# daihangpku/SW-NeRF

Measured on AMD Instinct MI355X. Metric: rays/sec (64+128 samples/ray), higher is better.
Workload: dtype f32

## Files before the change

### __graft_entry__.py

```python
import os
import subprocess
import sys

ROOT = os.path.dirname(os.path.abspath(__file__))
PKG = os.path.join(ROOT, "sw-nerf_amd")
CSRC = os.path.join(PKG, "csrc")
LIB = os.path.join(PKG, "swnerf", "libswnerf_hip.so")
SOURCES = ["render_kernels.hip", "train_kernels.hip", "misc_kernels.hip", "pack_kernels.hip", "backward_kernels.hip", "wgrad_kernels.hip", "wgrad_x3_kernels.hip", "generic_kernels.hip", "x3_kernels.hip", "mesh_kernels.hip", "tnerf_kernels.hip", "tnerf_train_kernels.hip", "metrics_kernels.hip", "pyramid_kernels.hip", "fit2d_kernels.hip", "batch_kernels.hip", "optim_kernels.hip", "patch_kernels.hip", "query_kernels.hip", "image_kernels.hip", "lpips_kernels.hip", "jpeg_kernels.hip", "jpeg_enc_kernels.hip", "marker_kernels.hip", "meshops_kernels.hip", "meshsimp_kernels.hip", "meshfill_kernels.hip"]
HEADERS = ["swnerf_common.h", "mlp_core.h", "mlp_core_x3.h", "bf16x3_split.h", "mlp_kernels.h", "render_pass.h", "composite.h", "resample.h", "wave_dpp.h", "lds_dma.h", "host_util.h", "wgrad_host.h", "mc_tables.h", "elu.h", "ray_rows.h", "tnerf_pass.h", "pyramid_interp.h", "jpeg_math.h", "jpeg_host.h", "jpeg_enc_math.h", "jpeg_enc_host.h", "marker_math.h", "meshops_math.h", "meshops_layout.h", "meshops_common.h", "par_prims.h", "fit2d_cols.h", os.path.join(ROOT, "include", "swnerf.h")]
HIPCC_FLAGS = ["--offload-arch=gfx950", "-O3", "-ffp-contract=off", "-fPIC", "-shared", "-std=c++17"]


OBJDIR = os.path.join(PKG, "build")


def _deps():
    return [os.path.join(CSRC, s) for s in SOURCES] + [h if os.path.isabs(h) else os.path.join(CSRC, h) for h in HEADERS]


def _stale():
    if not os.path.exists(LIB):
        return True
    t = os.path.getmtime(LIB)
    return any(os.path.getmtime(d) > t for d in _deps())


def compile_library(force=False):
    if not (force or _stale()):
        return False
    from concurrent.futures import ThreadPoolExecutor
    hipcc = os.environ.get("HIPCC", "/opt/rocm/bin/hipcc")
    os.makedirs(OBJDIR, exist_ok=True)
    newest_header = max(os.path.getmtime(h if os.path.isabs(h) else os.path.join(CSRC, h)) for h in HEADERS)
    jobs = []
    for s in SOURCES:
        src, obj = os.path.join(CSRC, s), os.path.join(OBJDIR, s.replace(".hip", ".o"))
        if force or not os.path.exists(obj) or os.path.getmtime(obj) < max(os.path.getmtime(src), newest_header):
            jobs.append([hipcc] + [f for f in HIPCC_FLAGS if f != "-shared"] + ["-c", src, "-o", obj])
    for cmd in jobs:
        print("[build]", " ".join(cmd), file=sys.stderr, flush=True)
    with ThreadPoolExecutor(max_workers=min(len(jobs), 6) or 1) as ex:
        for r in ex.map(lambda c: subprocess.run(c, cwd=CSRC), jobs):
            if r.returncode != 0:
                raise RuntimeError(f"hipcc failed: {' '.join(r.args)}")
    tmp = LIB + f".tmp{os.getpid()}"
    link = [hipcc, "--offload-arch=gfx950", "-fPIC", "-shared", "-o", tmp] + [os.path.join(OBJDIR, s.replace(".hip", ".o")) for s in SOURCES]
    print("[build]", " ".join(link), file=sys.stderr, flush=True)
    try:
        subprocess.run(link, check=True, cwd=CSRC)
        os.replace(tmp, LIB)
    finally:
        if os.path.exists(tmp):
            os.remove(tmp)
    return True


def compile_library_locked(force=False):
    if not (force or _stale()):
        return False
    import fcntl
    os.makedirs(OBJDIR, exist_ok=True)
    with open(os.path.join(OBJDIR, ".lock"), "w") as lk:
        fcntl.flock(lk, fcntl.LOCK_EX)
        try:
            return compile_library(force)
        finally:
            fcntl.flock(lk, fcntl.LOCK_UN)


def check_library():
    if _stale():
        raise RuntimeError(f"{LIB} is missing or older than its sources: run __graft_entry__.compile_library() before touching the GPU")
    if PKG not in sys.path:
        sys.path.insert(0, PKG)
    import swnerf
    from swnerf import _lib
    L = _lib.lib()
    missing = [n for n in _lib.EXPORTS if not hasattr(L, n)]
    if missing:
        raise RuntimeError(f"libswnerf_hip.so lacks symbols: {missing}")
    return L


def build(force=False):
    compile_library_locked(force)
    L = check_library()
    if ROOT not in sys.path:
        sys.path.insert(0, ROOT)
    import oracle.nerf_oracle
    print(f"[build] ok: {LIB} (version {L.swnerf_version()})", file=sys.stderr, flush=True)


# ... 49 lines not shown
```

### sw-nerf_amd/csrc/mlp_core.h

```cpp
#pragma once
#include <hip/hip_runtime.h>
#include "swnerf_common.h"
#include "lds_dma.h"

typedef float f32x16 __attribute__((ext_vector_type(16)));
typedef float f32x4 __attribute__((ext_vector_type(4)));

struct WStream {
    const char* base;
    unsigned voff;
    unsigned lds_addr;
    const float* ring;
    f32x4 a_cur;
    const float* bias;
    const char* cont;
};

template <int N>
__device__ __forceinline__ void ws_wait() {
    asm volatile("s_waitcnt vmcnt(%0)" :: "n"(N) : "memory");
}

__device__ __forceinline__ f32x4 ws_read(const WStream& ws, int slot) {
    return *reinterpret_cast<const f32x4*>(ws.ring + slot * SW_STEP_FLOATS);
}

template <int I>
__device__ __forceinline__ void ws_prime(WStream& ws) {
    if constexpr (I < SW_RING) {
        ws_dma(ws.base + I * 1024, ws.voff, ws.lds_addr + I * 1024);
        ws_prime<I + 1>(ws);
    }
}

__device__ __forceinline__ void ws_start(WStream& ws, const float* w, const float* lds_bias, float* lds_ring, int lane) {
    ws.base = reinterpret_cast<const char*>(w);
    ws.voff = (unsigned)lane * 16u;
    ws.lds_addr = __builtin_amdgcn_readfirstlane((unsigned)(size_t)lds_ring);
    ws.ring = lds_ring + lane * 4;
    ws.bias = lds_bias + (lane >> 5) * 16;
    ws_prime<0>(ws);
    ws_wait<SW_RING - 1>();
    ws.a_cur = ws_read(ws, 0);
}

__device__ __forceinline__ void ws_rewind(WStream& ws, const float* w, const float* lds_bias, int lane) {
    ws.base = reinterpret_cast<const char*>(w);
    ws.bias = lds_bias + (lane >> 5) * 16;
}

__device__ __forceinline__ void ws_restart(WStream& ws, const float* w) {
    asm volatile("s_waitcnt vmcnt(0)" ::: "memory");
    ws.base = reinterpret_cast<const char*>(w);
    ws_prime<0>(ws);
    ws_wait<SW_RING - 1>();
    ws.a_cur = ws_read(ws, 0);
}

enum { SEG_ACC = 0, SEG_BIAS = 1, SEG_ZERO = 2, SEG_BIAS_SCALED = 3 };
template <int INIT>
__device__ __forceinline__ void seg_init_read(f32x16& b, const WStream& ws, int n) {
    if constexpr (INIT == SEG_BIAS || INIT == SEG_BIAS_SCALED) {
#pragma unroll
        for (int g = 0; g < 4; ++g) {
            const f32x4 v = *reinterpret_cast<const f32x4*>(ws.bias + n * SW_BIAS_TILE_FLOATS + 4 * g);
            b[4 * g + 0] = v[0]; b[4 * g + 1] = v[1]; b[4 * g + 2] = v[2]; b[4 * g + 3] = v[3];
        }
    }
}

struct SideStore {
    float* sp;
    float* mp; f32x4 mv;
};

struct SideFetch {
    const char* base; unsigned voff, lds_addr;
};

template <int S, int NS, int NT, int KT, int INIT, int SK, int FK = 0, bool REDIR = false>
__device__ __forceinline__ void seg_steps(f32x16 (&out)[NT], const f32x16 (&kin)[KT], WStream& ws, f32x16& binit, float scale,
                                          const SideStore& ss, const SideFetch& sf = SideFetch{nullptr, 0u, 0u}) {
    if constexpr (S < NS) {
        constexpr int n = S / (KT * 4), kt = (S / 4) % KT, q = S % 4;
        constexpr int slot = S % SW_RING, nslot = (S + 1) % SW_RING;
        constexpr bool tile_first = (S % (KT * 4)) == 0, tile_last = ((S + 1) % (KT * 4)) == 0;
        if constexpr (tile_first) {
            if constexpr (INIT == SEG_BIAS) out[n] = binit;
            else if constexpr (INIT == SEG_BIAS_SCALED) out[n] = binit * scale;
            else if constexpr (INIT == SEG_ZERO) {
#pragma unroll
                for (int r = 0; r < 16; ++r) out[n][r] = 0.f;
            }
        }
        ws_wait<SW_RING - 2>();
        const f32x4 a_next = ws_read(ws, nslot);
        if constexpr (tile_last && n + 1 < NT) seg_init_read<INIT>(binit, ws, n + 1);
        __builtin_amdgcn_sched_barrier(0);
        const f32x4 a = ws.a_cur;
        out[n] = __builtin_amdgcn_mfma_f32_32x32x2f32(a[0], kin[kt][4 * q + 0], out[n], 0, 0, 0);
        out[n] = __builtin_amdgcn_mfma_f32_32x32x2f32(a[1], kin[kt][4 * q + 1], out[n], 0, 0, 0);
        out[n] = __builtin_amdgcn_mfma_f32_32x32x2f32(a[2], kin[kt][4 * q + 2], out[n], 0, 0, 0);
        out[n] = __builtin_amdgcn_mfma_f32_32x32x2f32(a[3], kin[kt][4 * q + 3], out[n], 0, 0, 0);
        __builtin_amdgcn_sched_barrier(0);
        if constexpr (REDIR && S + SW_RING >= NS) ws_dma(ws.cont + (S + SW_RING - NS) * 1024, ws.voff, ws.lds_addr + slot * 1024);
        else ws_dma(ws.base + (S + SW_RING) * 1024, ws.voff, ws.lds_addr + slot * 1024);
        if constexpr (SK > 0) {
            constexpr int total = 4 * SK, every = NS / total;
            static_assert(every >= 1, "segment too short for its side stores");
            if constexpr (S % every == every - 1 && S / every < total) {
                constexpr int idx = S / every, n2 = idx / 4, g = idx % 4;
                const f32x4 v = {kin[n2][4 * g], kin[n2][4 * g + 1], kin[n2][4 * g + 2], kin[n2][4 * g + 3]};
                *reinterpret_cast<f32x4*>(ss.sp + 32 * n2 + 8 * g) = v;
            }
            if constexpr (S == 1) {
                if (ss.mp) *reinterpret_cast<f32x4*>(ss.mp) = ss.mv;
            }
            __builtin_amdgcn_sched_barrier(0);
        }
        if constexpr (FK > 0) {
            constexpr int ftotal = 4 * FK, fevery = (NS - SW_RING) / ftotal;
            static_assert(fevery >= 1, "segment too short for its side fetches");
            if constexpr (S % fevery == 0 && S / fevery < ftotal) {
                constexpr int c = S / fevery;
                ws_dma(sf.base + (32 * (c >> 2) + 8 * (c & 3)) * 4, sf.voff, sf.lds_addr + c * 1024);
            }
        }
        ws.a_cur = a_next;
        seg_steps<S + 1, NS, NT, KT, INIT, SK, FK, REDIR>(out, kin, ws, binit, scale, ss, sf);
    }
}

template <int NT, int KT, int INIT, int SK = 0, int FK = 0, bool REDIR = false>
__device__ __forceinline__ void seg_mfma(f32x16 (&out)[NT], const f32x16 (&kin)[KT], WStream& ws, float scale = 1.f,
                                         const SideStore& ss = SideStore{nullptr, nullptr, {0.f, 0.f, 0.f, 0.f}},
                                         const SideFetch& sf = SideFetch{nullptr, 0u, 0u}) {
    constexpr int NS = NT * KT * 4;
    static_assert(NS % SW_RING == 0, "segment must keep the ring phase");
    f32x16 binit;
    seg_init_read<INIT>(binit, ws, 0);
    seg_steps<0, NS, NT, KT, INIT, SK, FK, REDIR>(out, kin, ws, binit, scale, ss, sf);
    if (INIT == SEG_BIAS || INIT == SEG_BIAS_SCALED) ws.bias += NT * SW_BIAS_TILE_FLOATS;
    if constexpr (REDIR) ws.base = ws.cont;
    else ws.base += NS * 1024;
}

#define SW_MASK_LAYERS 9
#define SW_MASK_TILE_FLOATS (SW_MASK_LAYERS * 256)
template <int NT>
__device__ __forceinline__ f32x4 relu_bits(const f32x16 (&t)[NT]) {
    unsigned m[4] = {0u, 0u, 0u, 0u};
#pragma unroll
    for (int n = 0; n < NT; ++n)
#pragma unroll
        for (int r = 0; r < 16; ++r) {
            const int b = min(max(__float_as_int(t[n][r]), 0), 1);
            m[n >> 1] |= (unsigned)b << (16 * (n & 1) + r);
        }
    f32x4 v = {__uint_as_float(m[0]), __uint_as_float(m[1]), __uint_as_float(m[2]), __uint_as_float(m[3])};
    return v;
}

template <int NT>
__device__ __forceinline__ void mask_apply(const f32x4& mv, f32x16 (&t)[NT]) {
#pragma unroll
    for (int n = 0; n < NT; ++n)
#pragma unroll
        for (int r = 0; r < 16; ++r) {
            const int m = __float_as_int(mv[n >> 1]);
            const int keep = (m << (31 - (16 * (n & 1) + r))) >> 31;
            t[n][r] = __int_as_float(__float_as_int(t[n][r]) & keep);
        }
}

__device__ __forceinline__ float relu1(float x) {
    float y;
    asm("v_max_f32_e32 %0, 0, %1" : "=v"(y) : "v"(x));
    return y;
}

template <int NOUT, int NT>
__device__ __forceinline__ void head_valu(const f32x16 (&x)[NT], WStream& ws, float (&res)[NOUT]) {
#pragma unroll
    for (int o = 0; o < NOUT; ++o) {
        float acc = 0.f;
#pragma unroll
        for (int n = 0; n < NT; ++n)
#pragma unroll
            for (int g = 0; g < 4; ++g) {
                const f32x4 w = *reinterpret_cast<const f32x4*>(ws.bias + (o * NT + n) * SW_BIAS_TILE_FLOATS + 4 * g);
                acc = fmaf(w[0], x[n][4 * g + 0], acc); acc = fmaf(w[1], x[n][4 * g + 1], acc);
                acc = fmaf(w[2], x[n][4 * g + 2], acc); acc = fmaf(w[3], x[n][4 * g + 3], acc);
            }
        res[o] = acc + __shfl_xor(acc, 32, 64);
        asm volatile("" : "+v"(res[o]));
    }
    ws.bias += NOUT * NT * SW_BIAS_TILE_FLOATS;
}

template <int NT>
__device__ __forceinline__ void head_valu_rt(const f32x16 (&x)[NT], WStream& ws, int nout, float (&res)[5]) {
#pragma nounroll
    for (int o = 0; o < nout; ++o) {
        float acc = 0.f;
#pragma unroll
        for (int n = 0; n < NT; ++n)
#pragma unroll
            for (int g = 0; g < 4; ++g) {
                const f32x4 w = *reinterpret_cast<const f32x4*>(ws.bias + (o * NT + n) * SW_BIAS_TILE_FLOATS + 4 * g);
                acc = fmaf(w[0], x[n][4 * g + 0], acc); acc = fmaf(w[1], x[n][4 * g + 1], acc);
                acc = fmaf(w[2], x[n][4 * g + 2], acc); acc = fmaf(w[3], x[n][4 * g + 3], acc);
            }
        float v = acc + __shfl_xor(acc, 32, 64);
        asm volatile("" : "+v"(v));
        res[0] = o == 0 ? v : res[0]; res[1] = o == 1 ? v : res[1]; res[2] = o == 2 ? v : res[2];
        res[3] = o == 3 ? v : res[3]; res[4] = o == 4 ? v : res[4];
    }
    ws.bias += nout * NT * SW_BIAS_TILE_FLOATS;
}

template <int NT>
__device__ __forceinline__ void tiles_store(float* rowp, const f32x16 (&t)[NT]) {
#pragma unroll
    for (int n = 0; n < NT; ++n)
#pragma unroll
        for (int g = 0; g < 4; ++g) {
            f32x4 v = {t[n][4 * g], t[n][4 * g + 1], t[n][4 * g + 2], t[n][4 * g + 3]};
            *reinterpret_cast<f32x4*>(rowp + 32 * n + 8 * g) = v;
        }
}

__device__ __forceinline__ void bias_to_lds(float* lds_bias, const float* gbias, int nfloats) {
    for (int i = threadIdx.x * 4; i < nfloats; i += blockDim.x * 4)
        *reinterpret_cast<f32x4*>(lds_bias + i) = *reinterpret_cast<const f32x4*>(gbias + i);
    __syncthreads();
}

__device__ __forceinline__ void pe_pos(float x0, float x1, float x2, int h, f32x16 (&e)[2]) {
#pragma unroll
    for (int a = 0; a < 32; ++a) {
        float v;
        if (a < 30) {
            const int k = a / 3, c = a % 3;
            const float xc = (c == 0) ? x0 : ((c == 1) ? x1 : x2);
            v = sw_sin_or_cos(xc * (float)(1 << k), h);
        } else if (a == 30) {
            v = h ? x2 : x0;
        } else {
            v = h ? 0.f : x1;
        }
        e[a >> 4][a & 15] = v;
    }
}

__device__ __forceinline__ void pe_dir(float d0, float d1, float d2, int h, f32x16& e) {
#pragma unroll
    for (int a = 0; a < 16; ++a) {
        float v = 0.f;
        if (a < 12) {
            const int k = a / 3, c = a % 3;
            const float dc = (c == 0) ? d0 : ((c == 1) ? d1 : d2);
            v = sw_sin_or_cos(dc * (float)(1 << k), h);
        } else if (a == 12) {
            v = h ? d2 : d0;
        } else if (a == 13) {
            v = h ? 0.f : d1;
        }
        e[a] = v;
    }
}

__device__ __forceinline__ void pe_time(float t, int h, f32x16& e) {
#pragma unroll
    for (int a = 0; a < 16; ++a) {
        float v = 0.f;
        if (a < 10) v = sw_sin_or_cos(t * (float)(1 << a), h);
        else if (a == 10) v = h ? 0.f : t;
        e[a] = v;
    }
}

#define SW_EMB_LDS_FLOATS (3 * 16 * 64)
__device__ __forceinline__ void emb_park(float* lds_emb, int lane, const f32x16 (&e)[2]) {
#pragma unroll
    for (int a = 0; a < 32; ++a) lds_emb[a * 64 + lane] = e[a >> 4][a & 15];
}
__device__ __forceinline__ void emb_fetch(const float* lds_emb, int lane, f32x16 (&e)[2]) {
#pragma unroll
    for (int a = 0; a < 32; ++a) e[a >> 4][a & 15] = lds_emb[a * 64 + lane];
}

__device__ __forceinline__ void tile_park(float* lds_tile, int lane, const f32x16& e) {
#pragma unroll
    for (int a = 0; a < 16; ++a) lds_tile[a * 64 + lane] = e[a];
}
__device__ __forceinline__ void tile_fetch(const float* lds_tile, int lane, f32x16& e) {
#pragma unroll
    for (int a = 0; a < 16; ++a) e[a] = lds_tile[a * 64 + lane];
}

template <bool DNERF, bool TRAIN = false, bool XS = false, bool NOHEAD = false, bool TB = false, bool REDIR = false>
__device__ __forceinline__ void trunk_pass(const f32x16 (&emb)[2], float* lds_emb, float t, bool deform_pass, int h,
                                           f32x16 (&in)[8], f32x16 (&out)[8], float (&head)[3], WStream& ws,
                                           float* act_row = nullptr, float* mask_tile = nullptr, bool store_last = false,
                                           f32x4* mb = nullptr, float* xs_row = nullptr, const float* lds_tb = nullptr,
                                           const char* cont7 = nullptr) {
    static_assert(!REDIR || (!TRAIN && !DNERF && !NOHEAD), "the redirect serves the static inference pass");
    const int lane_ = threadIdx.x & 63;
    emb_park(lds_emb, lane_, emb);
    f32x4 mbits = {0.f, 0.f, 0.f, 0.f};
#pragma nounroll
    for (int l = 0; l < 8; ++l) {
        if (l == 0) {
            if (DNERF && deform_pass) {
                if constexpr (TB) {
                    const float* keep = ws.bias;
                    ws.bias = lds_tb + (lane_ & 32 ? 16 : 0);
                    if (XS) {
                        seg_mfma<8, 2, SEG_BIAS, 2>(out, emb, ws, 1.f, SideStore{xs_row, nullptr, mbits});
                        f32x16 tt;
                        pe_time(t, h, tt);
#pragma unroll
                        for (int g = 0; g < 4; ++g) {
                            const f32x4 v = {tt[4 * g], tt[4 * g + 1], tt[4 * g + 2], tt[4 * g + 3]};
                            *reinterpret_cast<f32x4*>(xs_row + 64 + 8 * g) = v;
                        }
                    } else {
                        seg_mfma<8, 2, SEG_BIAS>(out, emb, ws);
                    }
                    ws.bias = keep;
                } else {
                    f32x16 k1[1];
                    pe_time(t, h, k1[0]);
                    seg_mfma<8, 1, SEG_BIAS>(out, k1, ws);
                    seg_mfma<8, 2, SEG_ACC>(out, emb, ws);
                }
            } else if (XS) {
                seg_mfma<8, 2, SEG_BIAS, 2>(out, emb, ws, 1.f, SideStore{xs_row, nullptr, mbits});
            } else {
                seg_mfma<8, 2, SEG_BIAS>(out, emb, ws);
            }
        } else {
            if (TRAIN) {
                const SideStore ss{act_row + 256 * (l - 1), mask_tile + 256 * (l - 1), mbits};
                seg_mfma<8, 8, SEG_BIAS, TRAIN ? 8 : 0>(out, in, ws, 1.f, ss);
            } else if constexpr (REDIR) {
                const char* next = ws.base + SW_STEPS_TRUNK * 1024;
                ws.cont = (l == 7 && cont7) ? cont7 : next;
                seg_mfma<8, 8, SEG_BIAS, 0, 0, true>(out, in, ws);
            } else {
                seg_mfma<8, 8, SEG_BIAS>(out, in, ws);
            }
            if (l == 5) {
                f32x16 e2[2];
                emb_fetch(lds_emb, lane_, e2);
                seg_mfma<8, 2, SEG_ACC>(out, e2, ws);
            }
        }
#pragma unroll
        for (int n = 0; n < 8; ++n)
#pragma unroll
            for (int r = 0; r < 16; ++r) in[n][r] = relu1(out[n][r]);
        if (TRAIN) mbits = relu_bits<8>(in);
    }
    if (TRAIN) {
        if (store_last) {
            tiles_store<8>(act_row + 256 * 7, in);
            *reinterpret_cast<f32x4*>(mask_tile + 256 * 7) = mbits;
        } else {
            *mb = mbits;
        }
    }
    if constexpr (NOHEAD) return;
    if (DNERF && deform_pass) {
        head_valu<3, 8>(in, ws, head);
        head[0] += ws.bias[0]; head[1] += ws.bias[1]; head[2] += ws.bias[2];
    } else {
        float s1[1];
        head_valu<1, 8>(in, ws, s1);
        head[0] = s1[0] + ws.bias[0]; head[1] = 0.f; head[2] = 0.f;
    }
    ws.bias += SW_BIAS_TILE_FLOATS;
}

#define SW_VB_LDS_FLOATS (4 * SW_BIAS_TILE_FLOATS)

__device__ __forceinline__ void view_bias_tile(const f32x16& demb, float* lds_vb, int lane, WStream& ws) {
    f32x16 k1[1], c[4];
    k1[0] = demb;
    seg_mfma<4, 1, SEG_BIAS>(c, k1, ws);
    if ((lane & 31) == 0) {
        float* o = lds_vb + (lane >> 5) * 16;
#pragma unroll
        for (int n = 0; n < 4; ++n)
#pragma unroll
            for (int g = 0; g < 4; ++g) {
                const f32x4 v = {c[n][4 * g], c[n][4 * g + 1], c[n][4 * g + 2], c[n][4 * g + 3]};
                *reinterpret_cast<f32x4*>(o + n * SW_BIAS_TILE_FLOATS + 4 * g) = v;
            }
    }
    __builtin_amdgcn_fence(__ATOMIC_ACQ_REL, "wavefront");
    __builtin_amdgcn_wave_barrier();
}

#define SW_TB_LDS_FLOATS (8 * SW_BIAS_TILE_FLOATS)
__device__ __forceinline__ void time_bias_tile(float t, int h, float* lds_tb, int lane, WStream& ws) {
    f32x16 k1[1], c[8];
    pe_time(t, h, k1[0]);
    seg_mfma<8, 1, SEG_BIAS>(c, k1, ws);
    if ((lane & 31) == 0) {
        float* o = lds_tb + (lane >> 5) * 16;
#pragma unroll
        for (int n = 0; n < 8; ++n)
#pragma unroll
            for (int g = 0; g < 4; ++g) {
                const f32x4 v = {c[n][4 * g], c[n][4 * g + 1], c[n][4 * g + 2], c[n][4 * g + 3]};
                *reinterpret_cast<f32x4*>(o + n * SW_BIAS_TILE_FLOATS + 4 * g) = v;
            }
    }
    __builtin_amdgcn_fence(__ATOMIC_ACQ_REL, "wavefront");
    __builtin_amdgcn_wave_barrier();
// ... 49 lines not shown
```

### sw-nerf_amd/csrc/render_pass.h

```cpp
#pragma once
#include <cstdlib>
#include "mlp_kernels.h"
#include "mlp_core_x3.h"
#include "resample.h"
#include "composite.h"
#include "ray_rows.h"

#define SW_LDS_SC 256
#define SW_LDS_SORT 1024
#define SW_LDS_WAVE_FLOATS (3 * SW_LDS_SC + SW_LDS_SORT)

#define SW_DEFER_SMAX 240
#define SW_DEFER_LDS_FLOATS (4 * SW_DEFER_SMAX + 64)
#define SW_DEFER_WS_FLOATS (64 * 256)
static_assert(SW_DEFER_LDS_FLOATS <= SW_LDS_SORT, "the deferred colour scratch shares the sort region");

struct PassDev {
    swnerf_pass_args a;
    const float* w0;
    const float* b0;
    int nbias;
    int two_pass;
    int sort_n, sort_s;
    float* act;
    float* bits;
    float* xs;
    float* act_d; float* bits_d; float* xs_d;
    int dir_steps;
    int time_steps;
    int tb_off;
    int warm_steps;
    int warm_blocks;
    int skew_mode;
    int skew_unit;
    float* view_ws;
};

__device__ __forceinline__ float wave32_sum(float v) {
#pragma unroll
    for (int o = 16; o > 0; o >>= 1) v += __shfl_xor(v, o, 32);
    return v;
}

__device__ __forceinline__ float z_linear(const swnerf_pass_args& a, float near, float far, int s) {
    const float t = sw_linspace(0.f, 1.f, a.n_samples, s);
    if (!a.lindisp) return near * (1.f - t) + far * t;
    return 1.f / (1.f / near * (1.f - t) + 1.f / far * t);
}

__device__ __forceinline__ float z_sample(const swnerf_pass_args& a, int64_t ray, float near, float far, int s) {
    const int S = a.n_samples;
    if (a.z_vals) return a.z_vals[ray * S + s];
    const float zs = z_linear(a, near, far, s);
    if (!a.t_rand) return zs;
    const float upper = (s < S - 1) ? .5f * (z_linear(a, near, far, s + 1) + zs) : zs;
    const float lower = (s > 0) ? .5f * (zs + z_linear(a, near, far, s - 1)) : zs;
    return lower + (upper - lower) * a.t_rand[ray * S + s];
}

#define SW_WARM_MAX_PER_WAVE 48
__device__ __forceinline__ void pass_startup(const PassDev& P, const float* w0, float* junk, int lane, int wv) {
    const unsigned b = blockIdx.x;
    if (P.warm_steps > 0 && (int)(b >> 3) < P.warm_blocks) {
        const unsigned junk_addr = __builtin_amdgcn_readfirstlane((unsigned)(size_t)junk);
        const int stride = P.warm_blocks * 4;
        int s = (int)(b >> 3) * 4 + wv;
#pragma nounroll
        for (int i = 0; i < SW_WARM_MAX_PER_WAVE && s < P.warm_steps; ++i, s += stride)
            ws_dma(reinterpret_cast<const char*>(w0) + (size_t)s * 1024, (unsigned)lane * 16u, junk_addr);
    }
    if (P.skew_mode) {
        const int k = (P.skew_mode == 1 ? (int)(b >> 3) : (int)(b >> 3) * 4 + wv) & 15;
#pragma nounroll
        for (int i = 0; i < k; ++i) __builtin_amdgcn_s_sleep(4);
        (void)P.skew_unit;
    }
}

static inline void pass_startup_args(PassDev& P, unsigned grid_x, int steps) {
    const char* ew = getenv("SWNERF_WARM");
    const char* es = getenv("SWNERF_SKEW");
    const int env_warm = ew ? atoi(ew) : 1, env_skew = es ? atoi(es) : 2;
    const unsigned first_round = grid_x < 256u ? grid_x : 256u;
    P.warm_blocks = (int)(first_round / 8u);
    P.warm_steps = (env_warm && P.warm_blocks > 0) ? steps + SW_TAIL : 0;
    P.skew_mode = env_skew;
    P.skew_unit = 4;
}

struct PassAccepts {
    const char* name;
    unsigned cols[4];
    int shape_code;
    const char* shape_msg;
    bool time_band;
    int smax;
};
#define SW_COLS(c) (1u << (c))

static inline int pass_check(const PassAccepts& e, const swnerf_pass_args& a) {
    if (!a.packed || (!a.ray_batch && a.n_rays != 0)) return sw_fail(SWNERF_E_ARG, e.smax ? "%s: NULL pointer" : "%s: NULL ray_batch/packed", e.name);
    if (a.kind < 0 || a.kind > 3 || a.cols < 0 || a.cols > 31 || !(e.cols[a.kind] >> a.cols & 1u)) return sw_fail(e.shape_code, e.shape_msg, e.name, a.cols, a.kind);
    if (e.smax && (a.n_rays < 0 || a.n_samples < 2 || a.n_samples > e.smax))
        return sw_fail(SWNERF_E_UNSUPP, "%s: 2 <= n_samples <= %d (got %d)", e.name, e.smax, a.n_samples);
    if (a.n_rays < 0 || a.n_samples < 2) return sw_fail(SWNERF_E_ARG, "%s: n_rays %lld, n_samples %d", e.name, (long long)a.n_rays, a.n_samples);
    if (a.L_pos < 0 || a.L_pos > 10 || a.L_dir < 0 || a.L_dir > 4 || (e.time_band && (a.L_time < 0 || a.L_time > 10)))
        return e.time_band ? sw_fail(SWNERF_E_UNSUPP, "%s: embedder bands (%d,%d,%d) exceed (10,4,10)", e.name, a.L_pos, a.L_dir, a.L_time)
                           : sw_fail(SWNERF_E_UNSUPP, "%s: embedder bands (%d,%d) exceed (10,4)", e.name, a.L_pos, a.L_dir);
    if (a.z_vals && a.t_rand) return sw_fail(SWNERF_E_ARG, "%s: t_rand only applies to coarse sampling", e.name);
    return 0;
}

static inline PassDev pass_dev(const swnerf_pass_args& a) {
    PassDev P = {};
    P.a = a;
    return P;
}

static inline int pass_resampling(const char* name, const swnerf_pass_args& a, PassDev& P, size_t& lds) {
// ... 68 lines not shown
    static constexpr int TRAIN_TILES = SW_NOVIEW_BIAS_TILES(SW_NOVIEW_MAX_OUT) > SW_CANON_BIAS_TILES ? SW_NOVIEW_BIAS_TILES(SW_NOVIEW_MAX_OUT) : SW_CANON_BIAS_TILES;
    static constexpr int BIAS = (TRAIN && !DNERF) ? TRAIN_TILES * SW_BIAS_TILE_FLOATS : SW_LDS_BIAS_FLOATS;
    static constexpr int FIXED = BIAS + 4 * SW_LDS_RING_FLOATS;
};
template <bool DNERF> struct X3Lds {
    static constexpr int BIAS = (DNERF ? SW_DEFORM_BIAS_TILES + SW_X3_CANON_BIAS_TILES : SW_X3_CANON_BIAS_TILES) * SW_BIAS_TILE_FLOATS;
    static constexpr int DIR = DNERF ? 0 : 16 * 64;
    static constexpr int WAVE = DIR + SW_ZSLOT_FLOATS;
    static constexpr int FIXED = BIAS + X3_RING_FLOATS + 4 * WAVE;
};

template <bool DNERF, bool TRAIN = false, int PREC = 0, bool VIEWS = true>
__global__ void __launch_bounds__(256, 1) render_pass_kernel(PassDev P) {
    static_assert(PREC == 0 || !TRAIN, "the bf16 paths cover the inference passes");
    static_assert(VIEWS || (!DNERF && PREC == 0), "the no-view-direction variant is a static fp32 pass (inference or TRAIN)");
    extern __shared__ __attribute__((aligned(16))) float lds_all[];
    const swnerf_pass_args& a = P.a;
    const int lane = threadIdx.x & 63, j = lane & 31, h = lane >> 5;
    const int wv = __builtin_amdgcn_readfirstlane(threadIdx.x >> 6);
    const int64_t ray_id = (int64_t)blockIdx.x * 4 + wv;
    if constexpr (PREC == 0)
        pass_startup(P, P.w0, lds_all + PassLds<DNERF, TRAIN>::BIAS + wv * SW_LDS_RING_FLOATS + SW_RING * SW_STEP_FLOATS, lane, wv);
    bias_to_lds(lds_all, P.b0, P.nbias);
    const bool ghost = PREC != 0 && ray_id >= a.n_rays;
    if (PREC == 0 && ray_id >= a.n_rays) return;
    const int64_t ray = ghost ? a.n_rays - 1 : ray_id;
    const float* lds_bias = lds_all;
    float* lds_ring = PREC ? lds_all + X3Lds<DNERF>::BIAS
                           : lds_all + PassLds<DNERF, TRAIN>::BIAS + wv * SW_LDS_RING_FLOATS;
    float* lds_emb = lds_ring + SW_RING * SW_STEP_FLOATS;
    float* lds_x3w = lds_ring + X3_RING_FLOATS + wv * X3Lds<DNERF>::WAVE;
    float* lds_dir = PREC ? lds_x3w : lds_emb + 2 * 16 * 64;
    float* lds_vb = lds_emb + SW_EMB_LDS_FLOATS + SW_ZSLOT_FLOATS;
    const float* lds_tb = (DNERF && PREC == 0 && P.time_steps) ? lds_all + P.tb_off + wv * SW_TB_LDS_FLOATS : nullptr;
    float* lds = PREC ? lds_all + X3Lds<DNERF>::FIXED + wv * SW_LDS_WAVE_FLOATS
                      : lds_all + PassLds<DNERF, TRAIN>::FIXED + wv * SW_LDS_WAVE_FLOATS;
    float* zc = lds;
    float* wc = lds + SW_LDS_SC;
    float* cdf = lds + 2 * SW_LDS_SC;
    float* srt = lds + 3 * SW_LDS_SC;

    const int S = a.n_samples;
    const bool resample = a.n_importance > 0;
    const float* rb = a.ray_batch + ray * a.cols;
    const float ox = rb[0], oy = rb[1], oz = rb[2], dx = rb[3], dy = rb[4], dz = rb[5];
    const float near = rb[6], far = rb[7];
    const float ft = (a.cols == 12) ? rb[8] : 0.f;
    const float v0 = VIEWS ? rb[a.cols - 3] : 0.f, v1 = VIEWS ? rb[a.cols - 2] : 0.f, v2 = VIEWS ? rb[a.cols - 1] : 0.f;
    const float dnorm = row_dnorm(ox, oy, oz, dx, dy, dz, near, far, ft);

    WStream ws;
    XStream xs;
    if constexpr (PREC != 0) {
        if (!DNERF) {
            f32x16 demb;
            pe_dir(v0, v1, v2, h, demb);
            tile_park(lds_dir, lane, demb);
        }
        x3_start(xs, reinterpret_cast<const char*>(P.w0), lds_bias, lds_ring, lane, wv);
    } else {
        ws_start(ws, P.w0, lds_bias, lds_ring, lane);
        if constexpr (VIEWS) {
            f32x16 demb;
            pe_dir(v0, v1, v2, h, demb);
            if constexpr (TRAIN) tile_park(lds_dir, lane, demb);
            view_bias_tile(demb, lds_vb, lane, ws);
        }
        if constexpr (DNERF) {
            if (P.time_steps) time_bias_tile(ft, h, lds_all + P.tb_off + wv * SW_TB_LDS_FLOATS, lane, ws);
        }
    }

    const float* zrow = a.z_vals ? a.z_vals + ray * S : nullptr;
    const float* zslot = PREC ? lds_x3w + X3Lds<DNERF>::DIR : lds_emb + SW_EMB_LDS_FLOATS;
    const unsigned zslot_addr = __builtin_amdgcn_readfirstlane((unsigned)(size_t)zslot);
    float pr = 0.f, pg = 0.f, pb = 0.f, pd = 0.f, pa = 0.f;
    double Tc = 1.0;
    const int ntiles = (S + 31) >> 5;
    constexpr bool DEFER_OK = !DNERF && !TRAIN && PREC == 0 && VIEWS;
    const bool defer = DEFER_OK && P.view_ws != nullptr;
    float* dW = resample ? srt : lds_all + PassLds<DNERF, TRAIN>::FIXED + wv * SW_DEFER_LDS_FLOATS;
    float* dC = dW + SW_DEFER_SMAX;
    int* dIdx = reinterpret_cast<int*>(dW + 4 * SW_DEFER_SMAX);
    float* vrow = DEFER_OK ? P.view_ws + ray * SW_DEFER_WS_FLOATS + h * 128 : nullptr;
    const char* main_head = reinterpret_cast<const char*>(P.w0 + (P.dir_steps + P.time_steps) * SW_STEP_FLOATS);
    const char* viewsh_head = main_head + (SW_CANON_MAIN_STEPS - SW_STEPS_VIEWSH) * 1024;
    int pend = 0, wr = 0, rd = 0;
    if constexpr (DEFER_OK) {
        if (defer) {
            for (int i = lane; i < 3 * SW_DEFER_SMAX; i += 64) dC[i] = 0.f;
            wave_lds_sync();
        }
    }
#pragma nounroll
    for (int tile = 0; tile < ntiles || (DEFER_OK && pend > 0); ++tile) {
        const bool is_tile = !DEFER_OK || tile < ntiles;
        const bool flush = !defer || !is_tile || pend >= 32;
        const int s = tile * 32 + j;
        const bool live = s < S && !ghost;
        const int sc = live ? s : S - 1;
        float z, zn;
        if (zrow && tile > 0) {
            const float* zs = zslot + (tile & 1) * 64;
            z = zs[j];
            const float z1 = zs[j + 1];
            zn = (s + 1 < S) ? z1 : z;
        } else {
            z = z_sample(a, ray, near, far, sc);
            zn = (s + 1 < S) ? z_sample(a, ray, near, far, s + 1) : z;
        }
        if (zrow && tile + 1 < ntiles)
            lds_dma_dword(reinterpret_cast<const char*>(zrow), (unsigned)min(32 * (tile + 1) + lane, S - 1) * 4u,
                          zslot_addr + (unsigned)((tile + 1) & 1) * 256u);
        float px = ox + dx * z, py = oy + dy * z, pz = oz + dz * z;

        f32x16 emb[2], in[8], out[8];
        float head[3], rgb[3];
        float extra = 0.f;
        if (is_tile) pe_pos(px, py, pz, h, emb);
        if (DNERF && TRAIN) {
            const int64_t tix = ray * ntiles + tile, prow = tix * 32 + j;
            float* act_row = P.act + prow * SW_ACT_LD + 4 * h;
            float* mask_tile = P.bits + tix * SW_MASK_TILE_FLOATS + lane * 4;
            float* xs_row = P.xs + prow * SW_XS_LD + 4 * h;
            f32x4 mb = {0.f, 0.f, 0.f, 0.f};
            f32x16 demb;
#pragma nounroll
            for (int pass = 0; pass < 2; ++pass) {
                const bool dp = pass == 0;
                trunk_pass<true, true, true, false, true>(emb, lds_emb, ft, dp, h, in, out, head, ws,
                                             dp ? P.act_d + prow * SW_ACT_LD + 4 * h : act_row,
                                             dp ? P.bits_d + tix * SW_MASK_TILE_FLOATS + lane * 4 : mask_tile, dp, &mb,
                                             dp ? P.xs_d + prow * SW_XS_LD + 4 * h : xs_row, lds_tb);
                if (dp) {
                    const float ex = head[0], ey = head[1], ez = head[2];
                    if (live && h == 0) {
                        float* o = a.dx + (ray * S + s) * 3;
                        o[0] = ex; o[1] = ey; o[2] = ez;
                    }
                    px = px + ex; py = py + ey; pz = pz + ez;
                    pe_pos(px, py, pz, h, emb);
                    tile_fetch(lds_dir, lane, demb);
#pragma unroll
                    for (int g = 0; g < 4; ++g) {
                        const f32x4 v = {demb[4 * g], demb[4 * g + 1], demb[4 * g + 2], demb[4 * g + 3]};
                        *reinterpret_cast<f32x4*>(xs_row + 64 + 8 * g) = v;
                    }
                }
            }
            canon_tail_train(in, lds_vb, rgb, ws.bias - SW_BIAS_TILE_FLOATS, ws, act_row, mask_tile, mb);
        } else if (DNERF && PREC != 0) {
            if constexpr (DNERF && PREC != 0) {
#pragma nounroll
                for (int pass = P.two_pass ? 0 : 1; pass < 2; ++pass) {
                    x3_net_dn_pipe<PREC>(px, py, pz, ft, pass == 0, h, v0, v1, v2, head, rgb, xs);
                    if (pass == 0) {
                        const float ex = head[0], ey = head[1], ez = head[2];
                        if (a.dx && live && h == 0) {
                            float* o = a.dx + (ray * S + s) * 3;
                            o[0] = ex; o[1] = ey; o[2] = ez;
                        }
                        px = px + ex; py = py + ey; pz = pz + ez;
                    }
                }
                if (!P.two_pass && a.dx && live && h == 0) {
                    float* o = a.dx + (ray * S + s) * 3;
                    o[0] = 0.f; o[1] = 0.f; o[2] = 0.f;
                }
                x3_rewind(xs, P.two_pass ? SW_X3_DEFORM_CHUNKS + SW_X3_CANON_CHUNKS : SW_X3_CANON_CHUNKS, lds_bias, lane);
            }
        } else if (DNERF) {
#pragma nounroll
            for (int pass = P.two_pass ? 0 : 1; pass < 2; ++pass) {
                trunk_pass<true, false, false, false, true>(emb, lds_emb, ft, pass == 0, h, in, out, head, ws, nullptr, nullptr, false, nullptr, nullptr, lds_tb);
                if (pass == 0) {
                    const float ex = head[0], ey = head[1], ez = head[2];
                    if (a.dx && live && h == 0) {
                        float* o = a.dx + (ray * S + s) * 3;
                        o[0] = ex; o[1] = ey; o[2] = ez;
                    }
                    px = px + ex; py = py + ey; pz = pz + ez;
                    pe_pos(px, py, pz, h, emb);
                }
            }
            if (!P.two_pass && a.dx && live && h == 0) {
                float* o = a.dx + (ray * S + s) * 3;
                o[0] = 0.f; o[1] = 0.f; o[2] = 0.f;
            }
        } else if (TRAIN && !VIEWS) {
            const int64_t prow = (ray * ntiles + tile) * 32 + j;
            float* act_row = P.act + prow * SW_ACT_LD + 4 * h;
            float* mask_tile = P.bits + (ray * ntiles + tile) * SW_MASK_TILE_FLOATS + lane * 4;
            float* xs_row = P.xs + prow * SW_XS_LD + 4 * h;
            f32x4 mb = {0.f, 0.f, 0.f, 0.f};
            trunk_pass<false, true, true, true>(emb, lds_emb, 0.f, false, h, in, out, head, ws, act_row, mask_tile, true, &mb, xs_row);
            float o5[5] = {0.f, 0.f, 0.f, 0.f, 0.f};
            head_valu_rt<8>(in, ws, a.out_ch, o5);
            rgb[0] = o5[0] + ws.bias[0]; rgb[1] = o5[1] + ws.bias[1]; rgb[2] = o5[2] + ws.bias[2];
            head[0] = o5[3] + ws.bias[3]; head[1] = 0.f; head[2] = 0.f;
            extra = o5[4] + ws.bias[4];
        } else if (TRAIN) {
            const int64_t prow = (ray * ntiles + tile) * 32 + j;
            float* act_row = P.act + prow * SW_ACT_LD + 4 * h;
            float* mask_tile = P.bits + (ray * ntiles + tile) * SW_MASK_TILE_FLOATS + lane * 4;
            float* xs_row = P.xs + prow * SW_XS_LD + 4 * h;
            f32x4 mb = {0.f, 0.f, 0.f, 0.f};
            f32x16 demb;
            tile_fetch(lds_dir, lane, demb);
#pragma unroll
            for (int g = 0; g < 4; ++g) {
                const f32x4 v = {demb[4 * g], demb[4 * g + 1], demb[4 * g + 2], demb[4 * g + 3]};
                *reinterpret_cast<f32x4*>(xs_row + 64 + 8 * g) = v;
            }
            trunk_pass<false, true, true>(emb, lds_emb, 0.f, false, h, in, out, head, ws, act_row, mask_tile, false, &mb, xs_row);
            canon_tail_train(in, lds_vb, rgb, ws.bias - SW_BIAS_TILE_FLOATS, ws, act_row, mask_tile, mb);
        } else if constexpr (PREC != 0) {
            head[1] = 0.f; head[2] = 0.f;
            x3_canon_pipe<PREC>(px, py, pz, h, lds_dir, lane, head[0], rgb, xs);
            x3_rewind(xs, SW_X3_CANON_CHUNKS, lds_bias, lane);
        } else if constexpr (!VIEWS) {
            trunk_pass<false, false, false, true>(emb, lds_emb, 0.f, false, h, in, out, head, ws);
            float o5[5] = {0.f, 0.f, 0.f, 0.f, 0.f};
            const int nout = (a.out_ch == 5 && !a.raw) ? 4 : a.out_ch;
            head_valu_rt<8>(in, ws, nout, o5);
            ws.bias += (a.out_ch - nout) * 8 * SW_BIAS_TILE_FLOATS;
            rgb[0] = o5[0] + ws.bias[0]; rgb[1] = o5[1] + ws.bias[1]; rgb[2] = o5[2] + ws.bias[2];
            head[0] = o5[3] + ws.bias[3]; head[1] = 0.f; head[2] = 0.f;
            extra = o5[4] + ws.bias[4];
        } else if (is_tile) {
            trunk_pass<false, false, false, false, false, true>(emb, lds_emb, 0.f, false, h, in, out, head, ws, nullptr, nullptr, false,
                                                                nullptr, nullptr, nullptr, (flush || tile + 1 >= ntiles) ? nullptr : main_head);
        }

        const float sg_raw = is_tile ? head[0] : 0.f;
        float sg = sg_raw;
        if (a.noise) sg += a.noise[ray * S + sc];
        const float alpha = comp_alpha(sg, comp_dist(s + 1 < S, zn, z, dnorm), live && is_tile);
        float w = 0.f;
        if (is_tile) {
            w = alpha * comp_transmittance(excl_cumprod_shfl<32>(comp_survival(alpha), j), Tc);
            if (live) {
                if (a.weights && h == 0) a.weights[ray * S + s] = w;
                if (a.z_out && h == 0) a.z_out[ray * S + s] = z;
                if (resample && h == 0) { zc[s] = z; wc[s] = w; }
            }
            comp_accumulate_density(w, z, pd, pa);
        }

        int src_s = s;
        bool src_ok = live;
        if constexpr (DEFER_OK) {
            if (defer) {
                const bool lit = is_tile && live && (!(alpha == 0.f) || s == 0);
                const unsigned m = (unsigned)__ballot(lit);
                const unsigned below = (1u << j) - 1u;
                const int cnt = __builtin_amdgcn_readfirstlane(__popc(m));
                if (live && is_tile && h == 0) dW[s] = w;
                if (!flush) {
                    const int slot = (wr + __popc(m & below)) & 63;
                    if (lit) {
                        if (h == 0) dIdx[slot] = s;
                        float* q = vrow + slot * 256;
#pragma unroll
                        for (int c = 0; c < 32; ++c) {
                            const f32x4 v = {in[c >> 2][4 * (c & 3)], in[c >> 2][4 * (c & 3) + 1], in[c >> 2][4 * (c & 3) + 2], in[c >> 2][4 * (c & 3) + 3]};
                            *reinterpret_cast<f32x4*>(q + c * 4) = v;
                        }
                    }
                    wr += cnt; pend += cnt;
                } else {
                    const int room = 32 - cnt, nv = pend < room ? pend : room;
                    const int rank = __popc(~m & below);
                    src_ok = lit || rank < nv;
                    if (!lit && (rank < nv || !is_tile)) {
                        const int slot = (rd + (rank < nv ? rank : nv - 1)) & 63;
                        src_s = dIdx[slot];
                        const float* p = vrow + slot * 256;
#pragma unroll
                        for (int c = 0; c < 32; ++c) {
                            const f32x4 v = *reinterpret_cast<const f32x4*>(p + c * 4);
                            in[c >> 2][4 * (c & 3) + 0] = v[0]; in[c >> 2][4 * (c & 3) + 1] = v[1];
                            in[c >> 2][4 * (c & 3) + 2] = v[2]; in[c >> 2][4 * (c & 3) + 3] = v[3];
                        }
                    }
                    rd += nv; pend -= nv;
                    if (!is_tile) ws.bias = lds_bias + (SW_DIR_BIAS_TILES + 64 + 8 + 1) * SW_BIAS_TILE_FLOATS + h * 16;
                }
                wave_lds_sync();
            }
        }
        const bool drain_next = DEFER_OK && tile + 1 >= ntiles && pend > 0;
        if (!TRAIN && PREC == 0 && VIEWS) {
            if (flush) {
                if constexpr (DEFER_OK) ws.cont = drain_next ? viewsh_head : ws.base + SW_STEPS_VIEWSH * 1024;
                canon_tail<DEFER_OK>(in, lds_vb, rgb, ws.bias - SW_BIAS_TILE_FLOATS, ws);
            }
        }
        if constexpr (PREC == 0) {
            ws_rewind(ws, P.w0 + (P.dir_steps + P.time_steps) * SW_STEP_FLOATS,
                      lds_bias + ((P.dir_steps ? SW_DIR_BIAS_TILES : 0) + (P.time_steps ? 8 : 0)) * SW_BIAS_TILE_FLOATS, lane);
            if (drain_next) ws.base = viewsh_head;
        }

        const float c0 = rgb[0], c1 = rgb[1], c2 = rgb[2];
        if (DEFER_OK && defer) {
            if (flush && src_ok && h == 0) { dC[src_s] = c0; dC[SW_DEFER_SMAX + src_s] = c1; dC[2 * SW_DEFER_SMAX + src_s] = c2; }
            continue;
        }
        if (a.raw && live && h == 0) {
            if (!VIEWS && a.out_ch == 5) {
                float* o = a.raw + (ray * S + s) * 5;
                o[0] = c0; o[1] = c1; o[2] = c2; o[3] = sg_raw; o[4] = extra;
            } else {
                f32x4 r4 = {c0, c1, c2, sg_raw};
                *reinterpret_cast<f32x4*>(a.raw + (ray * S + s) * 4) = r4;
            }
        }
        comp_accumulate_colour(w, c0, c1, c2, pr, pg, pb);
    }

    if constexpr (DEFER_OK) {
        if (defer) {
            wave_lds_sync();
#pragma nounroll
            for (int t = 0; t < ntiles; ++t) {
                const int s = t * 32 + j;
                const int sc = s < S ? s : S - 1;
                const float w = s < S ? dW[sc] : 0.f;
                const float c0 = dC[sc], c1 = dC[SW_DEFER_SMAX + sc], c2 = dC[2 * SW_DEFER_SMAX + sc];
                comp_accumulate_colour(w, c0, c1, c2, pr, pg, pb);
            }
        }
    }
    pr = wave32_sum(pr); pg = wave32_sum(pg); pb = wave32_sum(pb);
    pd = wave32_sum(pd); pa = wave32_sum(pa);
    if (lane == 0 && !ghost) comp_write_maps(pr, pg, pb, pd, pa, a.white_bkgd, ray, a.rgb_map, a.disp_map, a.acc_map, a.depth_map);
    if (!resample || ghost) return;

    wave_lds_sync();
    const int Ni = a.n_importance;
    const double sm = wave_sample_pdf(wc + 1, S - 1, MidBins{zc}, a.u ? a.u + ray * Ni : nullptr, Ni, cdf, srt, lane);
    if (a.z_std) {
        const float sd = wave_zstd(sm, srt, Ni, lane);
        if (lane == 0) a.z_std[ray] = sd;
    }
    wave_rank_merge(zc, S, P.sort_s, srt, Ni, P.sort_n, a.z_fine + ray * (S + Ni), lane);
}
```

Before: 554,900.

## Overlap deferred-sample ring stores with next tile's MFMA trunk segment

Moves the spill of deferred lit-sample features to the global ring out of the composite step. The 32 f32x4 stores are now issued one chunk at a time, interleaved into the next tile's first trunk MFMA segment, so their latency hides behind matrix math. The ring layout changes to chunk-major, with lanes of the same chunk adjacent, for more coalesced accesses. The input tile array is carried across iterations, and the last tile now always flushes. This adds register pressure from the carried input array and sched_barriers that may constrain the compiler's scheduling.

Result: no change. 557,100 (median of 6 runs) (+0.4%).

```diff
diff --git a/__graft_entry__.py b/__graft_entry__.py
--- a/__graft_entry__.py
+++ b/__graft_entry__.py
@@ -7,7 +7,7 @@
 CSRC = os.path.join(PKG, "csrc")
 LIB = os.path.join(PKG, "swnerf", "libswnerf_hip.so")
 SOURCES = ["render_kernels.hip", "train_kernels.hip", "misc_kernels.hip", "pack_kernels.hip", "backward_kernels.hip", "wgrad_kernels.hip", "wgrad_x3_kernels.hip", "generic_kernels.hip", "x3_kernels.hip", "mesh_kernels.hip", "tnerf_kernels.hip", "tnerf_train_kernels.hip", "metrics_kernels.hip", "pyramid_kernels.hip", "fit2d_kernels.hip", "batch_kernels.hip", "optim_kernels.hip", "patch_kernels.hip", "query_kernels.hip", "image_kernels.hip", "lpips_kernels.hip", "jpeg_kernels.hip", "jpeg_enc_kernels.hip", "marker_kernels.hip", "meshops_kernels.hip", "meshsimp_kernels.hip", "meshfill_kernels.hip"]
-HEADERS = ["swnerf_common.h", "mlp_core.h", "mlp_core_x3.h", "bf16x3_split.h", "mlp_kernels.h", "render_pass.h", "composite.h", "resample.h", "wave_dpp.h", "lds_dma.h", "host_util.h", "wgrad_host.h", "mc_tables.h", "elu.h", "ray_rows.h", "tnerf_pass.h", "pyramid_interp.h", "jpeg_math.h", "jpeg_host.h", "jpeg_enc_math.h", "jpeg_enc_host.h", "marker_math.h", "meshops_math.h", "meshops_layout.h", "meshops_common.h", "par_prims.h", "fit2d_cols.h", os.path.join(ROOT, "include", "swnerf.h")]
+HEADERS = ["swnerf_common.h", "mlp_core.h", "mlp_core_x3.h", "bf16x3_split.h", "mlp_kernels.h", "render_pass.h", "composite.h", "resample.h", "wave_dpp.h", "lds_dma.h", "host_util.h", "wgrad_host.h", "mc_tables.h", "elu.h", "ray_rows.h", "tnerf_pass.h", "pyramid_interp.h", "jpeg_math.h", "jpeg_host.h", "jpeg_enc_math.h", "jpeg_enc_host.h", "marker_math.h", "meshops_math.h", "meshops_layout.h", "meshops_common.h", "par_prims.h", "fit2d_cols.h", "defer_ring.h", os.path.join(ROOT, "include", "swnerf.h")]
 HIPCC_FLAGS = ["--offload-arch=gfx950", "-O3", "-ffp-contract=off", "-fPIC", "-shared", "-std=c++17"]
 
 
diff --git a/sw-nerf_amd/csrc/defer_ring.h b/sw-nerf_amd/csrc/defer_ring.h
--- /dev/null
+++ b/sw-nerf_amd/csrc/defer_ring.h
@@ -0,0 +1,23 @@
+#pragma once
+#include "swnerf_common.h"
+
+#define SW_DEFER_SLOTS 64
+#define SW_DEFER_CHUNKS 32
+#define SW_DEFER_CHUNK_BYTES (SW_DEFER_SLOTS * 2 * 16)
+#define SW_DEFER_WS_FLOATS (SW_DEFER_SLOTS * 256)
+
+SW_HD unsigned defer_below(int j) { return (1u << j) - 1u; }
+
+SW_HD bool defer_turn_flushes(bool defer, bool is_tile, bool last_tile, int pend) {
+    return !defer || !is_tile || last_tile || pend >= 32;
+}
+
+SW_HD int defer_slot(int wr, unsigned m, int j) { return (wr + __builtin_popcount(m & defer_below(j))) & (SW_DEFER_SLOTS - 1); }
+
+SW_HD int defer_fill_rank(unsigned m, int j) { return __builtin_popcount(~m & defer_below(j)); }
+SW_HD int defer_fill_count(int pend, int cnt) { return pend < 32 - cnt ? pend : 32 - cnt; }
+SW_HD bool defer_lane_loads(bool lit, int rank, int nv, bool is_tile) { return !lit && (rank < nv || !is_tile); }
+SW_HD int defer_fill_slot(int rd, int rank, int nv) { return (rd + (rank < nv ? rank : nv - 1)) & (SW_DEFER_SLOTS - 1); }
+
+SW_HD unsigned defer_lane_offset(int slot, int h) { return (unsigned)slot * 32u + (unsigned)h * 16u; }
+SW_HD unsigned defer_offset(int c, int slot, int h) { return (unsigned)c * SW_DEFER_CHUNK_BYTES + defer_lane_offset(slot, h); }
diff --git a/sw-nerf_amd/csrc/mlp_core.h b/sw-nerf_amd/csrc/mlp_core.h
--- a/sw-nerf_amd/csrc/mlp_core.h
+++ b/sw-nerf_amd/csrc/mlp_core.h
@@ -2,6 +2,7 @@
 #include <hip/hip_runtime.h>
 #include "swnerf_common.h"
 #include "lds_dma.h"
+#include "defer_ring.h"
 
 typedef float f32x16 __attribute__((ext_vector_type(16)));
 typedef float f32x4 __attribute__((ext_vector_type(4)));
@@ -78,9 +79,38 @@
     const char* base; unsigned voff, lds_addr;
 };
 
-template <int S, int NS, int NT, int KT, int INIT, int SK, int FK = 0, bool REDIR = false>
+struct RingStore {
+    char* base; unsigned voff; bool lit;
+};
+template <int C, class T>
+__device__ __forceinline__ __attribute__((address_space(1))) T* ring_chunk_base(T* base) {
+    T* b = base + (C >> 1) * 2 * SW_DEFER_CHUNK_BYTES;
+    asm("" : "+s"(b));
+    return (__attribute__((address_space(1))) T*)b;
+}
+template <int C>
+__device__ __forceinline__ void ring_store_chunk(const RingStore& rs, const f32x16 (&side)[8]) {
+    constexpr int n2 = C / 4, g = C % 4;
+    if (rs.lit) {
+        const f32x4 v = {side[n2][4 * g], side[n2][4 * g + 1], side[n2][4 * g + 2], side[n2][4 * g + 3]};
+        unsigned voff = rs.voff;
+        asm("" : "+v"(voff));
+        *(__attribute__((address_space(1))) f32x4*)(ring_chunk_base<C>(rs.base) + (C & 1) * SW_DEFER_CHUNK_BYTES + voff) = v;
+    }
+}
+template <int C>
+__device__ __forceinline__ void ring_load_chunks(const char* base, unsigned voff, f32x16 (&in)[8]) {
+    if constexpr (C < SW_DEFER_CHUNKS) {
+        const f32x4 v = *(const __attribute__((address_space(1))) f32x4*)(ring_chunk_base<C>(base) + (C & 1) * SW_DEFER_CHUNK_BYTES + voff);
+        in[C >> 2][4 * (C & 3) + 0] = v[0]; in[C >> 2][4 * (C & 3) + 1] = v[1];
+        in[C >> 2][4 * (C & 3) + 2] = v[2]; in[C >> 2][4 * (C & 3) + 3] = v[3];
+        ring_load_chunks<C + 1>(base, voff, in);
+    }
+}
+
+template <int S, int NS, int NT, int KT, int INIT, int SK, int FK = 0, bool REDIR = false, class... RING>
 __device__ __forceinline__ void seg_steps(f32x16 (&out)[NT], const f32x16 (&kin)[KT], WStream& ws, f32x16& binit, float scale,
-                                          const SideStore& ss, const SideFetch& sf = SideFetch{nullptr, 0u, 0u}) {
+                                          const SideStore& ss, const SideFetch& sf = SideFetch{nullptr, 0u, 0u}, const RING&... ring) {
     if constexpr (S < NS) {
         constexpr int n = S / (KT * 4), kt = (S / 4) % KT, q = S % 4;
         constexpr int slot = S % SW_RING, nslot = (S + 1) % SW_RING;
@@ -126,20 +156,28 @@
                 ws_dma(sf.base + (32 * (c >> 2) + 8 * (c & 3)) * 4, sf.voff, sf.lds_addr + c * 1024);
             }
         }
+        if constexpr (sizeof...(RING) > 0) {
+            constexpr int revery = NS / SW_DEFER_CHUNKS;
+            static_assert(revery >= 1, "segment too short for its ring stores");
+            if constexpr (S % revery == revery - 1 && S / revery < SW_DEFER_CHUNKS) {
+                ring_store_chunk<S / revery>(ring...);
+                __builtin_amdgcn_sched_barrier(0);
+            }
+        }
         ws.a_cur = a_next;
-        seg_steps<S + 1, NS, NT, KT, INIT, SK, FK, REDIR>(out, kin, ws, binit, scale, ss, sf);
-    }
-}
-
-template <int NT, int KT, int INIT, int SK = 0, int FK = 0, bool REDIR = false>
+        seg_steps<S + 1, NS, NT, KT, INIT, SK, FK, REDIR>(out, kin, ws, binit, scale, ss, sf, ring...);
+    }
+}
+
+template <int NT, int KT, int INIT, int SK = 0, int FK = 0, bool REDIR = false, class... RING>
 __device__ __forceinline__ void seg_mfma(f32x16 (&out)[NT], const f32x16 (&kin)[KT], WStream& ws, float scale = 1.f,
                                          const SideStore& ss = SideStore{nullptr, nullptr, {0.f, 0.f, 0.f, 0.f}},
-                                         const SideFetch& sf = SideFetch{nullptr, 0u, 0u}) {
+                                         const SideFetch& sf = SideFetch{nullptr, 0u, 0u}, const RING&... ring) {
     constexpr int NS = NT * KT * 4;
     static_assert(NS % SW_RING == 0, "segment must keep the ring phase");
     f32x16 binit;
     seg_init_read<INIT>(binit, ws, 0);
-    seg_steps<0, NS, NT, KT, INIT, SK, FK, REDIR>(out, kin, ws, binit, scale, ss, sf);
+    seg_steps<0, NS, NT, KT, INIT, SK, FK, REDIR>(out, kin, ws, binit, scale, ss, sf, ring...);
     if (INIT == SEG_BIAS || INIT == SEG_BIAS_SCALED) ws.bias += NT * SW_BIAS_TILE_FLOATS;
     if constexpr (REDIR) ws.base = ws.cont;
     else ws.base += NS * 1024;
@@ -299,12 +337,13 @@
     for (int a = 0; a < 16; ++a) e[a] = lds_tile[a * 64 + lane];
 }
 
-template <bool DNERF, bool TRAIN = false, bool XS = false, bool NOHEAD = false, bool TB = false, bool REDIR = false>
+template <bool DNERF, bool TRAIN = false, bool XS = false, bool NOHEAD = false, bool TB = false, bool REDIR = false, class... RING>
 __device__ __forceinline__ void trunk_pass(const f32x16 (&emb)[2], float* lds_emb, float t, bool deform_pass, int h,
                                            f32x16 (&in)[8], f32x16 (&out)[8], float (&head)[3], WStream& ws,
                                            float* act_row = nullptr, float* mask_tile = nullptr, bool store_last = false,
                                            f32x4* mb = nullptr, float* xs_row = nullptr, const float* lds_tb = nullptr,
-                                           const char* cont7 = nullptr) {
+                                           const char* cont7 = nullptr, const RING&... ring) {
+    static_assert(sizeof...(RING) == 0 || REDIR, "the ring stores serve the static inference pass");
     static_assert(!REDIR || (!TRAIN && !DNERF && !NOHEAD), "the redirect serves the static inference pass");
     const int lane_ = threadIdx.x & 63;
     emb_park(lds_emb, lane_, emb);
@@ -337,6 +376,8 @@
                 }
             } else if (XS) {
                 seg_mfma<8, 2, SEG_BIAS, 2>(out, emb, ws, 1.f, SideStore{xs_row, nullptr, mbits});
+            } else if constexpr (sizeof...(RING) > 0) {
+                seg_mfma<8, 2, SEG_BIAS>(out, emb, ws, 1.f, SideStore{nullptr, nullptr, mbits}, SideFetch{nullptr, 0u, 0u}, ring..., in);
             } else {
                 seg_mfma<8, 2, SEG_BIAS>(out, emb, ws);
             }
diff --git a/sw-nerf_amd/csrc/render_pass.h b/sw-nerf_amd/csrc/render_pass.h
--- a/sw-nerf_amd/csrc/render_pass.h
+++ b/sw-nerf_amd/csrc/render_pass.h
@@ -5,6 +5,7 @@
 #include "resample.h"
 #include "composite.h"
 #include "ray_rows.h"
+#include "defer_ring.h"
 
 #define SW_LDS_SC 256
 #define SW_LDS_SORT 1024
@@ -12,7 +13,6 @@
 
 #define SW_DEFER_SMAX 240
 #define SW_DEFER_LDS_FLOATS (4 * SW_DEFER_SMAX + 64)
-#define SW_DEFER_WS_FLOATS (64 * 256)
 static_assert(SW_DEFER_LDS_FLOATS <= SW_LDS_SORT, "the deferred colour scratch shares the sort region");
 
 struct PassDev {
@@ -35,6 +35,12 @@
     int skew_unit;
     float* view_ws;
 };
+
+template <bool FIRST, class A, class B>
+__device__ __forceinline__ auto& pass_pick(A& a, B& b) {
+    if constexpr (FIRST) return a;
+    else return b;
+}
 
 __device__ __forceinline__ float wave32_sum(float v) {
 #pragma unroll
@@ -269,10 +275,13 @@
     float* dW = resample ? srt : lds_all + PassLds<DNERF, TRAIN>::FIXED + wv * SW_DEFER_LDS_FLOATS;
     float* dC = dW + SW_DEFER_SMAX;
     int* dIdx = reinterpret_cast<int*>(dW + 4 * SW_DEFER_SMAX);
-    float* vrow = DEFER_OK ? P.view_ws + ray * SW_DEFER_WS_FLOATS + h * 128 : nullptr;
+    char* ring_ws = DEFER_OK ? reinterpret_cast<char*>(P.view_ws + ray * SW_DEFER_WS_FLOATS) : nullptr;
     const char* main_head = reinterpret_cast<const char*>(P.w0 + (P.dir_steps + P.time_steps) * SW_STEP_FLOATS);
     const char* viewsh_head = main_head + (SW_CANON_MAIN_STEPS - SW_STEPS_VIEWSH) * 1024;
     int pend = 0, wr = 0, rd = 0;
+    unsigned st_m = 0u;
+    int st_wr = 0;
+    f32x16 in_carried[DEFER_OK ? 8 : 1];
     if constexpr (DEFER_OK) {
         if (defer) {
             for (int i = lane; i < 3 * SW_DEFER_SMAX; i += 64) dC[i] = 0.f;
@@ -282,7 +291,7 @@
 #pragma nounroll
     for (int tile = 0; tile < ntiles || (DEFER_OK && pend > 0); ++tile) {
         const bool is_tile = !DEFER_OK || tile < ntiles;
-        const bool flush = !defer || !is_tile || pend >= 32;
+        const bool flush = defer_turn_flushes(defer, is_tile, DEFER_OK && tile + 1 == ntiles, pend);
         const int s = tile * 32 + j;
         const bool live = s < S && !ghost;
         const int sc = live ? s : S - 1;
@@ -301,7 +310,8 @@
                           zslot_addr + (unsigned)((tile + 1) & 1) * 256u);
         float px = ox + dx * z, py = oy + dy * z, pz = oz + dz * z;
 
-        f32x16 emb[2], in[8], out[8];
+        f32x16 emb[2], in_turn[DEFER_OK ? 1 : 8], out[8];
+        f32x16 (&in)[8] = pass_pick<DEFER_OK>(in_carried, in_turn);
         float head[3], rgb[3];
         float extra = 0.f;
         if (is_tile) pe_pos(px, py, pz, h, emb);
@@ -415,8 +425,10 @@
             head[0] = o5[3] + ws.bias[3]; head[1] = 0.f; head[2] = 0.f;
             extra = o5[4] + ws.bias[4];
         } else if (is_tile) {
+            const RingStore rs{ring_ws, defer_lane_offset(defer_slot(st_wr, st_m, j), h), (st_m >> j & 1u) != 0u};
             trunk_pass<false, false, false, false, false, true>(emb, lds_emb, 0.f, false, h, in, out, head, ws, nullptr, nullptr, false,
-                                                                nullptr, nullptr, nullptr, (flush || tile + 1 >= ntiles) ? nullptr : main_head);
+                                                                nullptr, nullptr, nullptr, flush ? nullptr : main_head, rs);
+            st_m = 0u;
         }
 
         const float sg_raw = is_tile ? head[0] : 0.f;
@@ -440,35 +452,20 @@
             if (defer) {
                 const bool lit = is_tile && live && (!(alpha == 0.f) || s == 0);
                 const unsigned m = (unsigned)__ballot(lit);
-                const unsigned below = (1u << j) - 1u;
                 const int cnt = __builtin_amdgcn_readfirstlane(__popc(m));
                 if (live && is_tile && h == 0) dW[s] = w;
                 if (!flush) {
-                    const int slot = (wr + __popc(m & below)) & 63;
-                    if (lit) {
-                        if (h == 0) dIdx[slot] = s;
-                        float* q = vrow + slot * 256;
-#pragma unroll
-                        for (int c = 0; c < 32; ++c) {
-                            const f32x4 v = {in[c >> 2][4 * (c & 3)], in[c >> 2][4 * (c & 3) + 1], in[c >> 2][4 * (c & 3) + 2], in[c >> 2][4 * (c & 3) + 3]};
-                            *reinterpret_cast<f32x4*>(q + c * 4) = v;
-                        }
-                    }
+                    if (lit && h == 0) dIdx[defer_slot(wr, m, j)] = s;
+                    st_m = m; st_wr = wr;
                     wr += cnt; pend += cnt;
                 } else {
-                    const int room = 32 - cnt, nv = pend < room ? pend : room;
-                    const int rank = __popc(~m & below);
+                    const int nv = defer_fill_count(pend, cnt);
+                    const int rank = defer_fill_rank(m, j);
                     src_ok = lit || rank < nv;
-                    if (!lit && (rank < nv || !is_tile)) {
-                        const int slot = (rd + (rank < nv ? rank : nv - 1)) & 63;
+                    if (defer_lane_loads(lit, rank, nv, is_tile)) {
+                        const int slot = defer_fill_slot(rd, rank, nv);
                         src_s = dIdx[slot];
-                        const float* p = vrow + slot * 256;
-#pragma unroll
-                        for (int c = 0; c < 32; ++c) {
-                            const f32x4 v = *reinterpret_cast<const f32x4*>(p + c * 4);
-                            in[c >> 2][4 * (c & 3) + 0] = v[0]; in[c >> 2][4 * (c & 3) + 1] = v[1];
-                            in[c >> 2][4 * (c & 3) + 2] = v[2]; in[c >> 2][4 * (c & 3) + 3] = v[3];
-                        }
+                        ring_load_chunks<0>(ring_ws, defer_lane_offset(slot, h), in);
                     }
                     rd += nv; pend -= nv;
                     if (!is_tile) ws.bias = lds_bias + (SW_DIR_BIAS_TILES + 64 + 8 + 1) * SW_BIAS_TILE_FLOATS + h * 16;
```
